# twitu/genome-assembly

Measured on NVIDIA B200. Metric: canonical k-mers binned+pruned per second, higher is better.
Workload: dtype u64

## Files before the change

genome-assembly_b200/csrc/bin3.cu:

```cuda
#include "bin3.cuh"
#include "gbin_device.cuh"
#include "gbin_internal.h"
#include "prefix_scan.cuh"

namespace gbin {


__device__ __forceinline__ uint32_t payload_bases(const uint32_t *pl, uint32_t nwords, uint32_t j, uint32_t h, bool rev) {
    const uint32_t bit = 2 * j, wi = bit >> 5, sh = bit & 31;
    const uint32_t a = wi < nwords ? pl[wi] : 0u, b = wi + 1 < nwords ? pl[wi + 1] : 0u;
    uint32_t x = __funnelshift_l(b, a, sh);
    if (rev) x = ~x;
    return h ? (x >> (32 - 2 * h)) : 0u;
}

template <int PW>
__global__ void __launch_bounds__(256)
    make_entries_kernel(const uint32_t *__restrict__ skr, uint64_t n_rec, KeyLayout kl, uint64_t *__restrict__ ent, uint16_t *__restrict__ piece_info,
                        unsigned long long *__restrict__ n_real) {
    constexpr int NW = SkrLayout<PW>::WORDS;
    const uint64_t i = (uint64_t)blockIdx.x * blockDim.x + threadIdx.x;
    uint32_t real = 0;
    if (i < n_rec) {
        const uint4 h = *reinterpret_cast<const uint4 *>(skr + i * NW);
// ... 293 lines not shown
                    emit(d - 1);
                    rnd++;
                    lo = d;
                    before += acc;
                    acc = 0;
                }
                acc += c;
            }
            emit(63);
            for (uint32_t j = rnd + 1; j < un.rounds; j++) {
                units[u + j].n_inst = 0;
                units[u + j].ibase = un.ibase + un.n_inst;
            }
            if (bad) atomicExch(&gc->overflow, 1u);
        }
        __syncwarp();
    }
}


struct UnitOut3 {
    uint32_t ibase;
    uint32_t S, N;
    uint32_t pad;
};

struct G3Stage {
    uint64_t *codes;
    uint32_t *mmer;
    uint32_t *loff;
    int32_t *ids;
    UnitOut3 *unit_out;
    uint64_t kmer_cap, id_cap;
    uint32_t kdiv;
};

template <int PW>
struct Payload {
    uint64_t w[PW];
    __device__ __forceinline__ void set(const uint4 &a, const uint4 &b) {
        w[0] = ((uint64_t)a.x << 32) | a.y;
        w[1] = ((uint64_t)a.z << 32) | a.w;
        if (PW == 4) {
            w[PW - 2] = ((uint64_t)b.x << 32) | b.y;
            w[PW - 1] = ((uint64_t)b.z << 32) | b.w;
        }
    }
    __device__ __forceinline__ void advance(uint32_t bases) {
        const uint32_t sh = 2 * bases;
#pragma unroll
        for (int q = 0; q < PW - 1; q++) w[q] = (w[q] << sh) | (w[q + 1] >> (64 - sh));
        w[PW - 1] <<= sh;
    }
    __device__ __forceinline__ void skip(uint32_t bases) {
        while (bases >= 31) {
            advance(31);
            bases -= 31;
        }
        if (bases) advance(bases);
    }
};

template <int PW, int KW>
__device__ __forceinline__ void front_kmer(const Payload<PW> &pl, int K, bool rev, uint64_t kmask0, uint64_t *k0, uint64_t *k1) {
    if (KW == 1) {
        uint64_t a = (2 * K == 64) ? pl.w[0] : (pl.w[0] >> (64 - 2 * K));
        if (rev) a = ~a & kmask0;
        *k0 = a;
        *k1 = 0;
    } else {
        const int r = 128 - 2 * K;
        uint64_t a = r ? (pl.w[0] >> r) : pl.w[0];
        uint64_t b = r ? ((pl.w[1] >> r) | (pl.w[0] << (64 - r))) : pl.w[1];
        if (rev) {
            a = ~a & kmask0;
            b = ~b;
        }
        *k0 = a;
        *k1 = b;
    }
}

template <int WCAP, int KW>
struct WarpLayout {
    static constexpr int NB_MAX = WCAP / 8;
    static constexpr int ECAP = WCAP / 4;
    static constexpr int BSTART_BYTES = ((NB_MAX + 1) * 2 + 15) / 16 * 16;
    static constexpr int BYTES = KW * WCAP * 8  + WCAP * 4  + WCAP * 2  + WCAP * 2  + WCAP * 2  + WCAP  + BSTART_BYTES +
                                 NB_MAX * 4  + ECAP * 4  + ECAP ;
};

__device__ __forceinline__ uint32_t warp_incl_scan_u32(uint32_t v, uint32_t lane) {
#pragma unroll
    for (int d = 1; d < 32; d <<= 1) {
        const uint32_t o = __shfl_up_sync(0xffffffffu, v, d);
        if (lane >= (uint32_t)d) v += o;
    }
    return v;
}

constexpr int G3_WARPS = 5;
constexpr uint32_t G3_SMALL_INST = 512, G3_SMALL_ENT = 128, G3_SMALL_NB = 64;

template <int PW, int KW, int WCAP, int WARPS, int U>
__global__ void __launch_bounds__(WARPS * 32)
    group3_kernel(const uint32_t *__restrict__ skr, const uint64_t *__restrict__ ent, const Unit3 *__restrict__ units, KeyLayout kl, int cutoff,
                  const int32_t *__restrict__ ids_by_arrival, int32_t id_base, G3Stage out, G3Counters *__restrict__ gc,
                  const uint32_t *__restrict__ chunk_bounds, uint32_t chunk, uint32_t *__restrict__ chunk_tickets, uint32_t size_class) {
    constexpr int NW = SkrLayout<PW>::WORDS;
    constexpr int HS = 2 * WCAP;
    constexpr int LOG_HS = WCAP == 512 ? 10 : 11;
    static_assert(WCAP == 512 || WCAP == 1024, "unit capacity");
    static_assert((1 << LOG_HS) == HS, "hash size");
    using WL = WarpLayout<WCAP, KW>;
    constexpr int NB_MAX = WL::NB_MAX, ECAP = WL::ECAP;
    extern __shared__ __align__(16) uint8_t smem3[];
    const uint32_t lane = threadIdx.x & 31, warp = threadIdx.x >> 5;
    uint8_t *wb = smem3 + (size_t)warp * WL::BYTES;
    uint64_t *key0 = reinterpret_cast<uint64_t *>(wb);
    uint64_t *key1 = key0 + (KW == 2 ? WCAP : 0);
    uint16_t *tbl16 = reinterpret_cast<uint16_t *>(key0 + KW * WCAP);
    uint32_t *cnt32 = reinterpret_cast<uint32_t *>(tbl16 + 2 * WCAP);
    uint16_t *cnt16 = reinterpret_cast<uint16_t *>(cnt32);
    uint16_t *grp = cnt16 + WCAP;
    uint16_t *rk = grp + WCAP;
    uint8_t *eix = reinterpret_cast<uint8_t *>(rk + WCAP);
    uint16_t *bstart = reinterpret_cast<uint16_t *>(eix + WCAP);
    uint32_t *bmm = reinterpret_cast<uint32_t *>(reinterpret_cast<uint8_t *>(bstart) + WL::BSTART_BYTES);
    int32_t *eid = reinterpret_cast<int32_t *>(bmm + NB_MAX);
    uint8_t *ebk = reinterpret_cast<uint8_t *>(eid + ECAP);
    uint16_t *surv = tbl16;
    uint16_t *sorted = surv + WCAP;
    int32_t *idbuf = reinterpret_cast<int32_t *>(tbl16);

    const int K = kl.K;
    const uint64_t kmask0 = (2 * K >= 64 * KW) ? ~0ull : ((1ull << (2 * K - 64 * (KW - 1))) - 1);
    const uint32_t unit_begin = chunk_bounds[chunk], unit_end = chunk_bounds[chunk + 1];
    const uint32_t lt_mask = (1u << lane) - 1u;
    const uint32_t cls_mask = (uint32_t)(kl.nc - 1);

    uint32_t u = 0;
    if (lane == 0) u = unit_begin + atomicAdd(&chunk_tickets[chunk], 1u);
    u = __shfl_sync(0xffffffffu, u, 0);
    while (u < unit_end) {
        Unit3 un;
        {
            const uint32_t wv = lane < 8 ? reinterpret_cast<const uint32_t *>(units + u)[lane] : 0u;
            un.ent_begin = __shfl_sync(0xffffffffu, wv, 0);
            un.ent_end = __shfl_sync(0xffffffffu, wv, 1);
            un.n_inst = __shfl_sync(0xffffffffu, wv, 2);
            un.round = __shfl_sync(0xffffffffu, wv, 3);
            un.rounds = __shfl_sync(0xffffffffu, wv, 4);
            un.drange = __shfl_sync(0xffffffffu, wv, 5);
            un.ibase = __shfl_sync(0xffffffffu, wv, 6);
        }
        uint32_t u_next = 0;
        if (lane == 0) u_next = unit_begin + atomicAdd(&chunk_tickets[chunk], 1u);
        const uint32_t u_cur = u;
        const bool is_round = un.rounds != 0;
        const uint32_t n_ent = un.ent_end - un.ent_begin;
        const bool packed = !is_round && n_ent <= (uint32_t)ECAP;
        if (size_class) {
            const bool small = !is_round && un.n_inst <= G3_SMALL_INST && n_ent <= G3_SMALL_ENT;
            if (small != (size_class == 1u)) {
                u = __shfl_sync(0xffffffffu, u_next, 0);
                continue;
            }
        }
        if (is_round && un.n_inst == 0) {
            if (lane == 0) out.unit_out[u_cur] = UnitOut3{un.ibase, 0u, 0u, 0u};
            u = __shfl_sync(0xffffffffu, u_next, 0);
            continue;
        }

        {
            uint4 *z = reinterpret_cast<uint4 *>(tbl16);
            for (uint32_t i = lane; i < (uint32_t)(WCAP * 4 + WCAP * 2) / 16; i += 32) z[i] = make_uint4(0u, 0u, 0u, 0u);
        }
        __syncwarp();

        int dlo = 0, dhi = 63;
        const uint32_t ibase = un.ibase;
        bool bad = false;
        if (is_round) {
            dlo = (int)(un.drange & 0xffu);
            dhi = (int)((un.drange >> 8) & 0xffu);
        }

        uint32_t n_inst = 0, n_bkt = 0;
        if (!bad) {
            uint32_t carry_pos = 0, carry_ord = 0, prev_mm = 0xffffffffu;
            for (uint32_t e0 = 0; e0 < n_ent; e0 += 32) {
                const uint32_t e = e0 + lane;
                uint32_t np = 0, t0 = 0, mm = 0xffffffffu, arrival = 0;
                bool rev = false;
                uint4 ha = make_uint4(0u, 0u, 0u, 0u), pa = ha, pb = ha;
                if (e < n_ent) {
                    const uint64_t en = ent[un.ent_begin + e];
                    const uint32_t slot = (uint32_t)en;
                    mm = (uint32_t)(en >> 32) >> kl.mshift;
                    const uint4 *rp = reinterpret_cast<const uint4 *>(skr + (uint64_t)(slot >> kl.cshift) * NW);
                    ha = rp[0];
                    pa = rp[1];
                    if (PW == 4) pb = rp[2];
                    arrival = ha.x;
                    const uint32_t meta = ha.z;
                    rev = (meta >> 8) & 1u;
                    piece_of(meta, slot & cls_mask, kl, &t0, &np);
                    if (is_round && np) {
                        const int so = (int)((meta >> 16) & 0xffu);
                        int a = so - dhi, b = so - dlo;
                        if (a < (int)t0) a = (int)t0;
                        if (b > (int)(t0 + np - 1)) b = (int)(t0 + np - 1);
                        if (dlo > dhi || b < a) np = 0;
                        else {
                            t0 = (uint32_t)a;
                            np = (uint32_t)(b - a + 1);
                        }
                    }
                }
                uint32_t pm = __shfl_up_sync(0xffffffffu, mm, 1);
                if (lane == 0) pm = prev_mm;
                const bool head = e < n_ent && mm != pm;
                const uint32_t hs = warp_incl_scan_u32(head ? 1u : 0u, lane);
                const uint32_t ps = warp_incl_scan_u32(np, lane);
                const uint32_t ord = carry_ord + hs - 1;
                const uint32_t pos0 = carry_pos + ps - np;
                if (head && ord < (uint32_t)NB_MAX) {
                    bstart[ord] = (uint16_t)pos0;
                    bmm[ord] = mm;
                }
                carry_ord += __shfl_sync(0xffffffffu, hs, 31);
                carry_pos += __shfl_sync(0xffffffffu, ps, 31);
                prev_mm = __shfl_sync(0xffffffffu, mm, 31);
                if (carry_pos > (uint32_t)WCAP || carry_ord > (uint32_t)NB_MAX || (!packed && carry_ord > 1u)) {
                    bad = true;
                    break;
                }
                if (packed && e < n_ent) {
                    eid[e] = ids_by_arrival ? ids_by_arrival[arrival] : id_base + (int32_t)arrival;
                    ebk[e] = (uint8_t)ord;
                }
                if (np) {
                    Payload<PW> pl;
                    pl.set(pa, pb);
                    pl.skip(t0);
                    for (uint32_t i = 0; i < np; i++) {
                        uint64_t k0, k1;
                        front_kmer<PW, KW>(pl, K, rev, kmask0, &k0, &k1);
                        key0[pos0 + i] = k0;
                        if (KW == 2) key1[pos0 + i] = k1;
                        if (packed) eix[pos0 + i] = (uint8_t)e;
                        pl.advance(1);
                    }
                }
            }
            n_inst = carry_pos;
            n_bkt = carry_ord;
            if (!bad && lane == 0) bstart[n_bkt] = (uint16_t)n_inst;
        }
        __syncwarp();
        if (bad) {
            if (lane == 0) {
                atomicExch(&gc->overflow, 1u);
                out.unit_out[u_cur] = UnitOut3{ibase, 0u, 0u, 0u};
            }
            u = __shfl_sync(0xffffffffu, u_next, 0);
            continue;
        }

        for (uint32_t b0 = 0; b0 < n_inst; b0 += 32 * U) {
            uint64_t k0[U], k1[U];
            uint32_t lo[U], hi[U], idx[U], rep[U], cur[U];
            bool valid[U];
#pragma unroll
            for (int j = 0; j < U; j++) {
                const uint32_t p = b0 + j * 32 + lane;
                valid[j] = p < n_inst;
                k0[j] = valid[j] ? key0[p] : 0ull;
                k1[j] = (KW == 2 && valid[j]) ? key1[p] : 0ull;
                uint32_t o = 0;
                if (packed && valid[j]) o = ebk[eix[p]];
                lo[j] = bstart[o];
                hi[j] = bstart[o + 1];
                uint32_t hx = ((uint32_t)k0[j] * 0x9E3779B1u) ^ ((uint32_t)(k0[j] >> 32) * 0x85EBCA77u) ^ (o * 0xC2B2AE3Du);
                if (KW == 2) hx ^= ((uint32_t)k1[j] * 0x27D4EB2Fu) ^ ((uint32_t)(k1[j] >> 32) * 0x165667B1u);
                hx *= 0x9E3779B1u;
                idx[j] = hx >> (32 - LOG_HS);
                rep[j] = 0xffffffffu;
            }
#pragma unroll
            for (int j = 0; j < U; j++) cur[j] = valid[j] ? tbl16[idx[j]] : 0u;
#pragma unroll
            for (int j = 0; j < U; j++) {
                if (valid[j] && cur[j] == 0) {
                    const uint32_t p = b0 + j * 32 + lane;
                    const uint32_t old = atomicCAS(&tbl16[idx[j]], (unsigned short)0, (unsigned short)(p + 1));
                    if (old == 0) rep[j] = p;
                    else cur[j] = old;
                }
            }
#pragma unroll
            for (int j = 0; j < U; j++) {
                if (valid[j] && rep[j] == 0xffffffffu) {
                    const uint32_t r = cur[j] - 1;
                    if (r >= lo[j] && r < hi[j] && key0[r] == k0[j] && (KW == 1 || key1[r] == k1[j])) rep[j] = r;
                }
            }
#pragma unroll
            for (int j = 0; j < U; j++) {
                if (valid[j] && rep[j] == 0xffffffffu) {
                    const uint32_t p = b0 + j * 32 + lane;
                    uint32_t ix = (idx[j] + 1) & (HS - 1);
                    for (;;) {
                        uint32_t c = tbl16[ix];
                        if (c == 0) {
                            c = atomicCAS(&tbl16[ix], (unsigned short)0, (unsigned short)(p + 1));
                            if (c == 0) {
                                rep[j] = p;
                                break;
                            }
                        }
                        const uint32_t r = c - 1;
                        if (r >= lo[j] && r < hi[j] && key0[r] == k0[j] && (KW == 1 || key1[r] == k1[j])) {
                            rep[j] = r;
                            break;
                        }
                        ix = (ix + 1) & (HS - 1);
                    }
                }
            }
            unsigned peers[U];
            uint32_t c[U];
#pragma unroll
            for (int j = 0; j < U; j++) peers[j] = __match_any_sync(0xffffffffu, valid[j] ? rep[j] : (0x10000u + lane));
#pragma unroll
            for (int j = 0; j < U; j++) {
                c[j] = 0;
                if (valid[j] && (int)lane == __ffs(peers[j]) - 1) {
                    const uint32_t sh = 16u * (rep[j] & 1u);
                    c[j] = (atomicAdd(&cnt32[rep[j] >> 1], (uint32_t)__popc(peers[j]) << sh) >> sh) & 0xffffu;
                }
                __syncwarp();
            }
#pragma unroll
            for (int j = 0; j < U; j++) {
                c[j] = __shfl_sync(0xffffffffu, c[j], __ffs(peers[j]) - 1);
                if (valid[j]) {
                    const uint32_t p = b0 + j * 32 + lane;
                    grp[p] = (uint16_t)rep[j];
                    rk[p] = (uint16_t)(c[j] + __popc(peers[j] & lt_mask));
                }
            }
        }
        __syncwarp();

        uint32_t S = 0, N = 0, D = 0;
        for (uint32_t b0 = 0; b0 < n_inst; b0 += 32 * U) {
            bool leader[U];
            uint32_t c[U];
#pragma unroll
            for (int j = 0; j < U; j++) {
                const uint32_t p = b0 + j * 32 + lane;
                leader[j] = p < n_inst && grp[p] == p;
            }
#pragma unroll
            for (int j = 0; j < U; j++) c[j] = leader[j] ? cnt16[b0 + j * 32 + lane] : 0u;
#pragma unroll
            for (int j = 0; j < U; j++) {
                const uint32_t p = b0 + j * 32 + lane;
                const bool sv = leader[j] && (cutoff < 0 || c[j] > (uint32_t)cutoff);
                const unsigned lm = __ballot_sync(0xffffffffu, leader[j]), sm = __ballot_sync(0xffffffffu, sv);
                if (sv) surv[S + __popc(sm & lt_mask)] = (uint16_t)p;
                else if (leader[j]) cnt16[p] = 0xffffu;
                S += __popc(sm);
                D += __popc(lm);
                N += sv ? c[j] : 0u;
            }
        }
#pragma unroll
        for (int d = 16; d > 0; d >>= 1) N += __shfl_xor_sync(0xffffffffu, N, d);
        const uint64_t kbase = ibase / out.kdiv;
        const bool oob = (uint64_t)ibase + N > out.id_cap || kbase + S > out.kmer_cap;
        if (lane == 0) {
            out.unit_out[u_cur] = UnitOut3{ibase, oob ? 0u : S, oob ? 0u : N, 0u};
            atomicAdd(&gc->distinct, (unsigned long long)D);
            if (oob) atomicExch(&gc->overflow, 2u);
        }
        __syncwarp();
        if (oob) {
            u = __shfl_sync(0xffffffffu, u_next, 0);
            continue;
        }

        for (uint32_t x0 = 0; x0 < S; x0 += 32) {
            const uint32_t x = x0 + lane;
            if (x < S) {
                const uint32_t p = surv[x];
                uint32_t a = 0, a2 = S;
                if (n_bkt > 1) {
                    const uint32_t o = ebk[eix[p]];
                    const uint32_t blo = bstart[o], bhi = bstart[o + 1];
                    uint32_t b = S;
                    while (a < b) {
                        const uint32_t m = (a + b) >> 1;
                        if (surv[m] < blo) a = m + 1;
                        else b = m;
                    }
                    uint32_t b2 = S;
                    a2 = a;
                    while (a2 < b2) {
                        const uint32_t m = (a2 + b2) >> 1;
                        if (surv[m] < bhi) a2 = m + 1;
                        else b2 = m;
                    }
                }
                const uint64_t k0 = key0[p], k1 = (KW == 2) ? key1[p] : 0ull;
                uint32_t rank = a;
                for (uint32_t t = a; t < a2; t++) {
                    const uint32_t q = surv[t];
                    const uint64_t q0 = key0[q];
                    bool less = q0 < k0;
                    if constexpr (KW == 2) less = less || (q0 == k0 && key1[q] < k1);
                    rank += less ? 1u : 0u;
                }
                sorted[rank] = (uint16_t)p;
            }
        }
        __syncwarp();

        {
            uint32_t carry = 0;
            for (uint32_t x0 = 0; x0 < S; x0 += 32) {
                const uint32_t x = x0 + lane;
                const uint32_t p = x < S ? sorted[x] : 0u;
                const uint32_t c = x < S ? cnt16[p] : 0u;
                const uint32_t inc = warp_incl_scan_u32(c, lane);
                if (x < S) cnt16[p] = (uint16_t)(carry + inc);
                carry += __shfl_sync(0xffffffffu, inc, 31);
            }
        }
        __syncwarp();

        for (uint32_t x0 = 0; x0 < S; x0 += 32) {
            const uint32_t x = x0 + lane;
            if (x < S) {
                const uint32_t p = sorted[x];
                const uint32_t beg = x ? cnt16[sorted[x - 1]] : 0u;
                const uint64_t g = kbase + x;
                out.codes[g * KW] = key0[p];
                if (KW == 2) out.codes[g * KW + 1] = key1[p];
                out.mmer[g] = bmm[n_bkt > 1 ? ebk[eix[p]] : 0u];
                out.loff[g] = beg;
            }
        }
        __syncwarp();

        if (N) {
            if (packed) {
                for (uint32_t b0 = 0; b0 < n_inst; b0 += 32 * U) {
                    uint32_t end[U], r[U];
                    int32_t id[U];
#pragma unroll
                    for (int j = 0; j < U; j++) {
                        const uint32_t p = b0 + j * 32 + lane;
                        end[j] = 0xffffu;
                        r[j] = 0;
                        id[j] = 0;
                        if (p < n_inst) {
                            end[j] = cnt16[grp[p]];
                            r[j] = rk[p];
                            id[j] = eid[eix[p]];
                        }
                    }
#pragma unroll
                    for (int j = 0; j < U; j++)
                        if (end[j] != 0xffffu) idbuf[end[j] - 1u - r[j]] = id[j];
                }
            } else {
                uint32_t carry_pos = 0;
                for (uint32_t e0 = 0; e0 < n_ent; e0 += 32) {
                    const uint32_t e = e0 + lane;
                    uint32_t np = 0, arrival = 0;
                    if (e < n_ent) {
                        const uint32_t slot = (uint32_t)ent[un.ent_begin + e];
                        const uint32_t *rec = skr + (uint64_t)(slot >> kl.cshift) * NW;
                        const uint32_t meta = rec[2];
                        arrival = rec[0];
                        uint32_t t0;
                        piece_of(meta, slot & cls_mask, kl, &t0, &np);
                        if (is_round && np) {
                            const int so = (int)((meta >> 16) & 0xffu);
                            int a = so - dhi, b = so - dlo;
                            if (a < (int)t0) a = (int)t0;
                            if (b > (int)(t0 + np - 1)) b = (int)(t0 + np - 1);
                            np = (dlo > dhi || b < a) ? 0u : (uint32_t)(b - a + 1);
                        }
                    }
                    const uint32_t ps = warp_incl_scan_u32(np, lane);
                    const uint32_t pos0 = carry_pos + ps - np;
                    carry_pos += __shfl_sync(0xffffffffu, ps, 31);
                    if (np) {
                        const int32_t id = ids_by_arrival ? ids_by_arrival[arrival] : id_base + (int32_t)arrival;
                        for (uint32_t i = 0; i < np; i++) {
                            const uint32_t p = pos0 + i;
                            const uint32_t end = cnt16[grp[p]];
                            if (end != 0xffffu) idbuf[end - 1u - rk[p]] = id;
                        }
                    }
                }
            }
            __syncwarp();
            int32_t *dst = out.ids + ibase;
            for (uint32_t i = lane; i < N; i += 32) dst[i] = idbuf[i];
        }
        __syncwarp();
        u = __shfl_sync(0xffffffffu, u_next, 0);
    }
}


struct UnitSN {
    const UnitOut3 *uo;
    const uint32_t *chunk_bounds;
    uint32_t chunk;
    __device__ __forceinline__ uint64_t operator()(uint64_t u) const {
        if (u < chunk_bounds[chunk] || u >= chunk_bounds[chunk + 1]) return 0ull;
        return ((uint64_t)uo[u].S << 32) | uo[u].N;
    }
};

__global__ void v3_chunk_total_kernel(const uint64_t *__restrict__ chunk_sum, uint32_t chunk, unsigned long long *__restrict__ totals, G3Counters *__restrict__ gc,
                                      uint32_t n_chunks, int which) {
    const unsigned long long t = (chunk ? totals[chunk - 1] : 0ull) + *chunk_sum;
    totals[chunk] = t;
    if (chunk + 1 == n_chunks) {
        if (which == 0) {
            gc->total_kmers = t >> 32;
            gc->total_ids = t & 0xffffffffull;
        } else {
            gc->lsd_kmers = t >> 32;
            gc->lsd_ids = t & 0xffffffffull;
        }
    }
}

struct G3Final {
    uint64_t *kmer_codes;
    uint32_t *kmer_mmer;
    uint64_t *kmer_id_off;
    int32_t *read_ids;
    uint64_t id_off_base;
};

struct G3Lsd {
    const uint64_t *excl;
    void *rec;
    uint32_t *src_off;
    uint32_t *cnt;
    uint32_t *fidx;
    uint32_t *nadj;
    uint64_t cap;
};

struct UnitSNLong {
    const UnitOut3 *uo;
    const Unit3 *units;
    const uint32_t *chunk_bounds;
    uint32_t chunk;
    __device__ __forceinline__ uint64_t operator()(uint64_t u) const {
        if (u < chunk_bounds[chunk] || u >= chunk_bounds[chunk + 1]) return 0ull;
        const uint32_t sl = units[u].span_len;
        if (sl != SPAN_MEMBER_LONG && (sl <= SPAN_SHORT_MAX || sl == SPAN_MEMBER)) return 0ull;
        return ((uint64_t)uo[u].S << 32) | uo[u].N;
    }
};

template <int KW>
__device__ __forceinline__ void finalize3_unit(const Unit3 *__restrict__ units, const uint64_t *__restrict__ unit_excl, unsigned long long base,
                                               unsigned long long lsd_base, const G3Stage &st, const G3Final &fin, const G3Lsd &ls, G3Counters *gc, uint32_t u,
                                               uint32_t lane, bool only_long) {
    const uint32_t span_len = units[u].span_len;
    if (only_long && span_len != SPAN_MEMBER_LONG && (span_len <= SPAN_SHORT_MAX || span_len == SPAN_MEMBER)) return;
    const uint64_t ex = unit_excl[u];
    const UnitOut3 uo = st.unit_out[u];
    const uint64_t Sb = (base >> 32) + (ex >> 32), Nb = (base & 0xffffffffull) + (ex & 0xffffffffull);
    if (span_len == 0) {
        const uint64_t kb = uo.ibase / st.kdiv;
        for (uint32_t x0 = 0; x0 < uo.S; x0 += 128) {
            uint64_t c0[4], c1[4];
            uint32_t mm[4], lo[4];
#pragma unroll
            for (int q = 0; q < 4; q++) {
                const uint32_t x = x0 + q * 32 + lane;
                if (x < uo.S) {
                    c0[q] = st.codes[(kb + x) * KW];
                    if (KW == 2) c1[q] = st.codes[(kb + x) * KW + 1];
                    mm[q] = st.mmer[kb + x];
                    lo[q] = st.loff[kb + x];
                }
// ... 130 lines not shown
__global__ void lsd_place_kernel(const Rec<KW> *__restrict__ rec, uint64_t n, const uint64_t *__restrict__ dnew, G3Lsd ls, G3Final fin) {
    const uint64_t q = (uint64_t)blockIdx.x * blockDim.x + threadIdx.x;
    if (q >= n) return;
    const Rec<KW> r = load_rec<KW>(rec + q);
    const uint64_t f = ls.fidx[q];
    fin.kmer_codes[f * KW] = r.k[0];
    if (KW == 2) fin.kmer_codes[f * KW + 1] = r.k[KW - 1];
    fin.kmer_mmer[f] = r.mmer;
    fin.kmer_id_off[f] = fin.id_off_base + dnew[q] + ls.nadj[q];
}

template <int KW>
__global__ void __launch_bounds__(256)
    lsd_lists_kernel(const Rec<KW> *__restrict__ rec, uint64_t n, const uint64_t *__restrict__ dnew, G3Lsd ls, const int32_t *__restrict__ stg_ids, G3Final fin) {
    const uint64_t q = ((uint64_t)blockIdx.x * blockDim.x + threadIdx.x) >> 3;
    if (q >= n) return;
    const uint32_t p = rec[q].arrival;
    const uint32_t c = ls.cnt[p];
    const int32_t *src = stg_ids + ls.src_off[p];
    int32_t *dst = fin.read_ids + dnew[q] + ls.nadj[q];
    for (uint32_t i = threadIdx.x & 7u; i < c; i += 8) dst[i] = src[i];
}

__global__ void v3_chunk_bounds_kernel(const Unit3 *__restrict__ units, const G3Counters *__restrict__ gc, uint32_t n_chunks, uint32_t *__restrict__ chunk_bounds) {
    const uint32_t nu = gc->n_units;
    for (uint32_t c = 0; c <= n_chunks; c++) {
        uint32_t b = (uint32_t)(((uint64_t)nu * c) / n_chunks);
        if (c == n_chunks) b = nu;
        else {
            while (b > 0 && b < nu && (units[b].span_len == SPAN_MEMBER || units[b].span_len == SPAN_MEMBER_LONG)) b--;
        }
        chunk_bounds[c] = b;
    }
}


static bool v3_hybrid(const KeyLayout &kl, int cap_i) { return cap_i != 512 && kl.K <= 32; }
static Plan3 v3_plan_params(const KeyLayout &kl, int cap_i) {
    const uint32_t cap = cap_i == 512 ? 512u : 1024u;
    Plan3 pp{cap, cap / 8, cap / 4, (uint32_t)(kl.K - kl.M + 1), cap, cap / 8, cap / 4};
    if (v3_hybrid(kl, cap_i)) {
        pp.cap_s = G3_SMALL_INST;
        pp.nb_s = G3_SMALL_NB;
        pp.ecap_s = G3_SMALL_ENT;
    }
    return pp;
}

uint64_t v3_max_units(uint64_t n_inst, uint64_t n_runs, int cap) {
    const uint64_t c = cap == 512 ? 512 : 1024;
    return n_runs + 5 * (n_inst / c) + 16;
}
size_t v3_unit_bytes() { return sizeof(Unit3); }
size_t v3_unit_out_bytes() { return sizeof(UnitOut3); }

struct PtrIn64 {
    const uint64_t *p;
    __device__ __forceinline__ uint64_t operator()(uint64_t j) const { return p[j]; }
};

int v3_plan_units(const uint16_t *sorted_info, const uint64_t *ent, const KeyLayout &kl, int cap, const uint32_t *inst_prefix, const uint32_t *run_start, uint64_t n_runs,
                  uint64_t *nunits64, uint64_t *base64, uint32_t *atom3, uint32_t *spanlen, uint32_t *head_run, void *scratch, void *units, uint64_t max_units,
                  void *gc_dev, uint32_t n_chunks, uint32_t *chunk_bounds, cudaStream_t st) {
    RunView3 rv{run_start, inst_prefix};
    const Plan3 pp = v3_plan_params(kl, cap);
    G3Counters *gc = static_cast<G3Counters *>(gc_dev);
    cudaMemsetAsync(gc, 0, sizeof(G3Counters), st);
    int l = 0;
    if (n_runs) {
        uint32_t *atom_c = atom3, *atom_e = atom3 + n_runs, *atom_mm = atom3 + 2 * n_runs;
        v3_atoms_kernel<<<(unsigned)((n_runs + 255) / 256), 256, 0, st>>>(rv, ent, n_runs, kl.mshift, atom_c, atom_e, atom_mm);
        const uint64_t walkers = (n_runs + PLAN_BLOCK - 1) / PLAN_BLOCK;
        v3_pack_kernel<<<(unsigned)((walkers + 127) / 128), 128, 0, st>>>(atom_c, atom_e, atom_mm, n_runs, pp, nunits64, spanlen);
        l += 2 + exclusive_scan<uint64_t, PtrIn64>(PtrIn64{nunits64}, base64, n_runs, static_cast<uint64_t *>(scratch), base64 + n_runs, st);
        v3_head_runs_kernel<<<(unsigned)((n_runs + 255) / 256), 256, 0, st>>>(nunits64, base64, n_runs, head_run);
        v3_fill_units_kernel<<<(unsigned)((max_units + 255) / 256), 256, 0, st>>>(rv, nunits64, spanlen, base64, base64 + n_runs, n_runs, head_run, static_cast<Unit3 *>(units), gc);
        v3_round_cuts_kernel<<<592, 128, 0, st>>>(sorted_info, static_cast<Unit3 *>(units), gc, pp.cap);
        l += 3;
    }
    v3_chunk_bounds_kernel<<<1, 1, 0, st>>>(static_cast<const Unit3 *>(units), gc, n_chunks, chunk_bounds);
    return l + 1;
}

size_t v3_group_smem_bytes(int KW, int cap) {
    const size_t per_warp = cap == 512 ? (KW == 1 ? WarpLayout<512, 1>::BYTES : WarpLayout<512, 2>::BYTES)
                                       : (KW == 1 ? WarpLayout<1024, 1>::BYTES : WarpLayout<1024, 2>::BYTES);
    return per_warp * G3_WARPS;
}

int v3_group_launch(const void *skr, const uint64_t *ent, const void *units, const KeyLayout &kl, int cap, int cutoff, const int32_t *ids_by_arrival, int32_t id_base,
                    const V3Out &o, uint64_t max_units, uint64_t *unit_excl, uint64_t *lsd_excl, void *scan_scratch, void *gc_dev, const V3Chunks &ch, const V3Lsd &lsd,
                    bool finalize_only, int sm_count, KernelProf *prof, cudaStream_t st) {
    const int KW = kl.K <= 32 ? 1 : 2;
    constexpr int WARPS = G3_WARPS;
    const size_t smem = v3_group_smem_bytes(KW, cap);
    cudaMemsetAsync(ch.tickets, 0, sizeof(uint32_t) * 2 * ch.n, st);
    const uint32_t kdiv = cutoff >= 0 ? (uint32_t)cutoff + 1u : 1u;
    G3Stage stg{o.stg_codes, o.stg_mmer, o.stg_loff, o.stg_ids, static_cast<UnitOut3 *>(o.unit_out), o.kmer_cap, o.id_cap, kdiv};
    G3Final fin{o.kmer_codes, o.kmer_mmer, o.kmer_id_off, o.read_ids, o.id_off_base};
    G3Lsd ls{lsd_excl, lsd.rec, lsd.src_off, lsd.cnt, lsd.fidx, lsd.nadj, lsd.cap};
    G3Counters *gc = static_cast<G3Counters *>(gc_dev);
    const uint32_t *sk = static_cast<const uint32_t *>(skr);
    const Unit3 *un = static_cast<const Unit3 *>(units);
    int per_sm = (int)((size_t)(227 * 1024) / (smem + 1024));
    if (per_sm < 1) per_sm = 1;
    const bool hybrid = v3_hybrid(kl, cap);
    const size_t smem_s = v3_group_smem_bytes(KW, 512);
    int per_sm_s = (int)((size_t)(227 * 1024) / (smem_s + 1024));
    if (per_sm_s < 1) per_sm_s = 1;
    int launches = 0;
    auto launch = [&](auto kern, auto kern_small, auto fin_kern) {
        cudaFuncSetAttribute(kern, cudaFuncAttributeMaxDynamicSharedMemorySize, (int)smem);
        if (hybrid) cudaFuncSetAttribute(kern_small, cudaFuncAttributeMaxDynamicSharedMemorySize, (int)smem_s);
        for (uint32_t c = 0; c < ch.n; c++) {
            if (!finalize_only) {
                bool on = prof && prof->begin(KK_SKR_GROUP, st);
                if (!hybrid) {
                    kern<<<sm_count * per_sm, WARPS * 32, smem, st>>>(sk, ent, un, kl, cutoff, ids_by_arrival, id_base, stg, gc, ch.bounds, c, ch.tickets, 0u);
                } else {
                    cudaEventRecord(ch.ev_fork, st);
                    cudaStreamWaitEvent(ch.aux, ch.ev_fork, 0);
                    kern<<<sm_count * 2, WARPS * 32, smem, st>>>(sk, ent, un, kl, cutoff, ids_by_arrival, id_base, stg, gc, ch.bounds, c, ch.tickets, 2u);
                    kern_small<<<sm_count * per_sm_s, WARPS * 32, smem_s, ch.aux>>>(sk, ent, un, kl, cutoff, ids_by_arrival, id_base, stg, gc, ch.bounds, c, ch.tickets + ch.n, 1u);
                    cudaEventRecord(ch.ev_join, ch.aux);
                    cudaStreamWaitEvent(st, ch.ev_join, 0);
                }
                if (prof) prof->end(on, hybrid ? 2 : 1, st);
                launches += hybrid ? 2 : 1;
            }
            bool on = prof && prof->begin(KK_V3_SPAN, st);
            int l = exclusive_scan<uint64_t, UnitSN>(UnitSN{stg.unit_out, ch.bounds, c}, unit_excl, max_units, static_cast<uint64_t *>(scan_scratch), ch.chunk_sum, st);
            v3_chunk_total_kernel<<<1, 1, 0, st>>>(ch.chunk_sum, c, ch.totals_dev, gc, ch.n, 0);
            l += exclusive_scan<uint64_t, UnitSNLong>(UnitSNLong{stg.unit_out, un, ch.bounds, c}, lsd_excl, max_units, static_cast<uint64_t *>(scan_scratch), ch.chunk_sum, st);
            v3_chunk_total_kernel<<<1, 1, 0, st>>>(ch.chunk_sum, c, ch.lsd_totals_dev, gc, ch.n, 1);
            fin_kern<<<sm_count * 12, 128, 0, st>>>(un, unit_excl, ch.totals_dev, ch.lsd_totals_dev, stg, fin, ls, gc, ch.bounds, c, finalize_only);
            if (prof) prof->end(on, l + 3, st);
            launches += l + 3;
            if (ch.totals_host) {
                cudaMemcpyAsync(ch.totals_host + c, ch.totals_dev + c, sizeof(unsigned long long), cudaMemcpyDeviceToHost, st);
                cudaMemcpyAsync(ch.lsd_totals_host + c, ch.lsd_totals_dev + c, sizeof(unsigned long long), cudaMemcpyDeviceToHost, st);
            }
            if (ch.done) cudaEventRecord(ch.done[c], st);
        }
    };
    if (KW == 1) {
        if (cap == 512) launch(group3_kernel<2, 1, 512, WARPS, 2>, group3_kernel<2, 1, 512, WARPS, 2>, finalize3_kernel<1>);
        else launch(group3_kernel<2, 1, 1024, WARPS, 4>, group3_kernel<2, 1, 512, WARPS, 2>, finalize3_kernel<1>);
    } else {
        if (cap == 512) launch(group3_kernel<4, 2, 512, WARPS, 2>, group3_kernel<4, 2, 512, WARPS, 2>, finalize3_kernel<2>);
        else launch(group3_kernel<4, 2, 1024, WARPS, 4>, group3_kernel<4, 2, 512, WARPS, 2>, finalize3_kernel<2>);
    }
    return launches;
}

template <int KW>
struct RecHead {
    const Rec<KW> *rec;
    __device__ __forceinline__ uint32_t operator()(uint64_t p) const { return (p == 0 || rec[p].mmer != rec[p - 1].mmer) ? 1u : 0u; }
};
template <int KW>
__global__ void span_starts_kernel(const Rec<KW> *__restrict__ rec, uint64_t n, const uint32_t *__restrict__ idx, uint32_t *__restrict__ starts,
                                   uint32_t *__restrict__ n_spans, uint32_t *__restrict__ flag) {
    const uint64_t p = (uint64_t)blockIdx.x * blockDim.x + threadIdx.x;
    if (p >= n) return;
    const bool head = p == 0 || rec[p].mmer != rec[p - 1].mmer;
    if (head) starts[idx[p]] = (uint32_t)p;
    if (p == n - 1) {
        const uint32_t total = idx[p] + (head ? 1u : 0u);
        starts[total] = (uint32_t)n;
        *n_spans = total;
        *flag = 0u;
    }
}

constexpr int SS_RMAX = 1024;
template <int KW, int CAP, int THREADS>
__global__ void __launch_bounds__(THREADS)
    span_sort_kernel(Rec<KW> *__restrict__ rec, const uint32_t *__restrict__ starts, const uint32_t *__restrict__ n_spans_ptr, uint32_t m_min, uint32_t m_max,
                     uint32_t *__restrict__ too_big) {
    extern __shared__ __align__(16) uint8_t ss_smem[];
    uint64_t *ka = reinterpret_cast<uint64_t *>(ss_smem);
    uint64_t *kb = ka + KW * CAP;
    uint16_t *sa = reinterpret_cast<uint16_t *>(kb + KW * CAP);
    uint16_t *sb = sa + CAP;
    uint16_t *ra = sb + CAP;
    uint16_t *rb = ra + SS_RMAX + 2;
    __shared__ uint32_t s_nruns;
    const uint32_t tid = threadIdx.x, lane = tid & 31;
    const uint32_t n_spans = *n_spans_ptr;
    for (uint32_t s = blockIdx.x; s < n_spans; s += gridDim.x) {
        const uint32_t b = starts[s], m = starts[s + 1] - b;
        if (m < m_min) continue;
        if (m > m_max) continue;
        const uint32_t mmer = rec[b].mmer;
        for (uint32_t i = tid; i < m; i += THREADS) {
            const Rec<KW> r = load_rec<KW>(rec + b + i);
            ka[i] = r.k[0];
            if (KW == 2) ka[CAP + i] = r.k[KW - 1];
            sa[i] = (uint16_t)i;
        }
        __syncthreads();
        if (tid < 32) {
            uint32_t nr = 0;
            for (uint32_t i0 = 0; i0 < m; i0 += 32) {
                const uint32_t i = i0 + lane;
                bool head = false;
                if (i < m) {
                    head = i == 0 || ka[i] < ka[i - 1];
                    if (KW == 2 && i && ka[i] == ka[i - 1]) head = ka[CAP + i] < ka[CAP + i - 1];
                }
                const unsigned bal = __ballot_sync(0xffffffffu, head);
                if (head) {
                    const uint32_t pos = nr + __popc(bal & ((1u << lane) - 1u));
                    if (pos < (uint32_t)SS_RMAX) ra[pos] = (uint16_t)i;
                }
                nr += __popc(bal);
            }
            if (lane == 0) {
                s_nruns = nr;
                if (nr <= (uint32_t)SS_RMAX) ra[nr] = (uint16_t)m;
            }
        }
        __syncthreads();
        uint32_t nr = s_nruns;
        if (nr > (uint32_t)SS_RMAX) {
            if (tid == 0) atomicExch(too_big, 1u);
            __syncthreads();
            continue;
        }
        uint64_t *src_k = ka, *dst_k = kb;
        uint16_t *src_s = sa, *dst_s = sb, *src_r = ra, *dst_r = rb;
        while (nr > 1) {
            for (uint32_t i = tid; i < m; i += THREADS) {
// ... 307 lines not shown
```

Baseline: 23.41 billion.

## Process 1024-capacity group units with warp pairs instead of single warps

For the 1024-instance unit capacity, each unit is now handled by two cooperating warps synchronised with named barriers. Cross-warp scans and totals go through a small shared exchange buffer, and each warp keeps its own count table that is merged later. The hybrid large-class launch also changes from a fixed two CTAs per SM to the occupancy-derived CTA count. This aims to cut per-unit latency and raise parallelism on large units, at the cost of extra barriers, a second count table in shared memory, and fewer units per CTA.

```diff
diff --git a/genome-assembly_b200/csrc/bin3.cu b/genome-assembly_b200/csrc/bin3.cu
--- a/genome-assembly_b200/csrc/bin3.cu
+++ b/genome-assembly_b200/csrc/bin3.cu
@@ -399,12 +399,14 @@
 }
 
 template <int WCAP, int KW>
-struct WarpLayout {
+struct UnitLayout {
+    static constexpr int W = WCAP == 1024 ? 2 : 1;
     static constexpr int NB_MAX = WCAP / 8;
     static constexpr int ECAP = WCAP / 4;
     static constexpr int BSTART_BYTES = ((NB_MAX + 1) * 2 + 15) / 16 * 16;
-    static constexpr int BYTES = KW * WCAP * 8  + WCAP * 4  + WCAP * 2  + WCAP * 2  + WCAP * 2  + WCAP  + BSTART_BYTES +
-                                 NB_MAX * 4  + ECAP * 4  + ECAP ;
+    static constexpr int XCH_BYTES = W == 2 ? 64 : 0;
+    static constexpr int BYTES = KW * WCAP * 8  + WCAP * 4  + W * WCAP * 2  + WCAP * 2  + WCAP * 2  + WCAP  +
+                                 BSTART_BYTES + NB_MAX * 4  + ECAP * 4  + ECAP  + XCH_BYTES;
 };
 
 __device__ __forceinline__ uint32_t warp_incl_scan_u32(uint32_t v, uint32_t lane) {
@@ -416,36 +418,83 @@
     return v;
 }
 
+template <int W>
+__device__ __forceinline__ void unit_sync(uint32_t bar_id) {
+    if (W == 1) __syncwarp();
+    else asm volatile("bar.sync %0, 64;" ::"r"(bar_id) : "memory");
+}
+
+struct PairXch {
+    uint32_t *x;
+    uint32_t slot;
+    __device__ __forceinline__ const uint32_t *put(uint32_t h, uint32_t lane, uint32_t bar_id, uint32_t a, uint32_t b = 0u, uint32_t c = 0u) {
+        uint32_t *s = x + slot * 8;
+        if (lane == 0) {
+            s[h * 4] = a;
+            s[h * 4 + 1] = b;
+            s[h * 4 + 2] = c;
+        }
+        slot ^= 1u;
+        unit_sync<2>(bar_id);
+        return s;
+    }
+};
+
+template <int W>
+__device__ __forceinline__ uint32_t unit_incl_scan(uint32_t v, uint32_t lane, uint32_t h, uint32_t bar_id, PairXch &xc, uint32_t *total) {
+    v = warp_incl_scan_u32(v, lane);
+    const uint32_t wt = __shfl_sync(0xffffffffu, v, 31);
+    if (W == 1) {
+        *total = wt;
+        return v;
+    }
+    const uint32_t *s = xc.put(h, lane, bar_id, wt);
+    *total = s[0] + s[4];
+    return v + (h ? s[0] : 0u);
+}
+
 constexpr int G3_WARPS = 5;
+constexpr int G3_PAIRS = 3;
+constexpr int g3_ctas_per_sm(size_t smem) {
+    const int n = (int)((size_t)(227 * 1024) / (smem + 1024));
+    return n > 1 ? n : 1;
+}
 constexpr uint32_t G3_SMALL_INST = 512, G3_SMALL_ENT = 128, G3_SMALL_NB = 64;
 
-template <int PW, int KW, int WCAP, int WARPS, int U>
-__global__ void __launch_bounds__(WARPS * 32)
+template <int PW, int KW, int WCAP, int UNITS, int U>
+__global__ void __launch_bounds__(UNITS * UnitLayout<WCAP, KW>::W * 32, WCAP == 1024 ? g3_ctas_per_sm(UNITS * UnitLayout<WCAP, KW>::BYTES) : 0)
     group3_kernel(const uint32_t *__restrict__ skr, const uint64_t *__restrict__ ent, const Unit3 *__restrict__ units, KeyLayout kl, int cutoff,
                   const int32_t *__restrict__ ids_by_arrival, int32_t id_base, G3Stage out, G3Counters *__restrict__ gc,
                   const uint32_t *__restrict__ chunk_bounds, uint32_t chunk, uint32_t *__restrict__ chunk_tickets, uint32_t size_class) {
+    using WL = UnitLayout<WCAP, KW>;
+    constexpr int W = WL::W;
     constexpr int NW = SkrLayout<PW>::WORDS;
     constexpr int HS = 2 * WCAP;
     constexpr int LOG_HS = WCAP == 512 ? 10 : 11;
     static_assert(WCAP == 512 || WCAP == 1024, "unit capacity");
     static_assert((1 << LOG_HS) == HS, "hash size");
-    using WL = WarpLayout<WCAP, KW>;
     constexpr int NB_MAX = WL::NB_MAX, ECAP = WL::ECAP;
     extern __shared__ __align__(16) uint8_t smem3[];
     const uint32_t lane = threadIdx.x & 31, warp = threadIdx.x >> 5;
-    uint8_t *wb = smem3 + (size_t)warp * WL::BYTES;
+    const uint32_t h = warp % W, bar_id = 1 + warp / W;
+    const uint32_t ul = h * 32 + lane;
+    const bool first = ul == 0;
+    uint8_t *wb = smem3 + (size_t)(warp / W) * WL::BYTES;
     uint64_t *key0 = reinterpret_cast<uint64_t *>(wb);
     uint64_t *key1 = key0 + (KW == 2 ? WCAP : 0);
     uint16_t *tbl16 = reinterpret_cast<uint16_t *>(key0 + KW * WCAP);
     uint32_t *cnt32 = reinterpret_cast<uint32_t *>(tbl16 + 2 * WCAP);
     uint16_t *cnt16 = reinterpret_cast<uint16_t *>(cnt32);
-    uint16_t *grp = cnt16 + WCAP;
+    uint32_t *cntlo32 = cnt32 + (W - 1) * WCAP / 2;
+    uint16_t *cntlo16 = reinterpret_cast<uint16_t *>(cntlo32);
+    uint16_t *grp = cnt16 + W * WCAP;
     uint16_t *rk = grp + WCAP;
     uint8_t *eix = reinterpret_cast<uint8_t *>(rk + WCAP);
     uint16_t *bstart = reinterpret_cast<uint16_t *>(eix + WCAP);
     uint32_t *bmm = reinterpret_cast<uint32_t *>(reinterpret_cast<uint8_t *>(bstart) + WL::BSTART_BYTES);
     int32_t *eid = reinterpret_cast<int32_t *>(bmm + NB_MAX);
     uint8_t *ebk = reinterpret_cast<uint8_t *>(eid + ECAP);
+    PairXch xc{reinterpret_cast<uint32_t *>(ebk + ECAP), 0u};
     uint16_t *surv = tbl16;
     uint16_t *sorted = surv + WCAP;
     int32_t *idbuf = reinterpret_cast<int32_t *>(tbl16);
@@ -455,10 +504,14 @@
     const uint32_t unit_begin = chunk_bounds[chunk], unit_end = chunk_bounds[chunk + 1];
     const uint32_t lt_mask = (1u << lane) - 1u;
     const uint32_t cls_mask = (uint32_t)(kl.nc - 1);
+    auto share_ticket = [&](uint32_t t) -> uint32_t {
+        if (W == 1) return __shfl_sync(0xffffffffu, t, 0);
+        return xc.put(h, lane, bar_id, __shfl_sync(0xffffffffu, t, 0))[0];
+    };
 
     uint32_t u = 0;
-    if (lane == 0) u = unit_begin + atomicAdd(&chunk_tickets[chunk], 1u);
-    u = __shfl_sync(0xffffffffu, u, 0);
+    if (first) u = unit_begin + atomicAdd(&chunk_tickets[chunk], 1u);
+    u = share_ticket(u);
     while (u < unit_end) {
         Unit3 un;
         {
@@ -472,7 +525,7 @@
             un.ibase = __shfl_sync(0xffffffffu, wv, 6);
         }
         uint32_t u_next = 0;
-        if (lane == 0) u_next = unit_begin + atomicAdd(&chunk_tickets[chunk], 1u);
+        if (first) u_next = unit_begin + atomicAdd(&chunk_tickets[chunk], 1u);
         const uint32_t u_cur = u;
         const bool is_round = un.rounds != 0;
         const uint32_t n_ent = un.ent_end - un.ent_begin;
@@ -480,21 +533,21 @@
         if (size_class) {
             const bool small = !is_round && un.n_inst <= G3_SMALL_INST && n_ent <= G3_SMALL_ENT;
             if (small != (size_class == 1u)) {
-                u = __shfl_sync(0xffffffffu, u_next, 0);
+                u = share_ticket(u_next);
                 continue;
             }
         }
         if (is_round && un.n_inst == 0) {
-            if (lane == 0) out.unit_out[u_cur] = UnitOut3{un.ibase, 0u, 0u, 0u};
-            u = __shfl_sync(0xffffffffu, u_next, 0);
+            if (first) out.unit_out[u_cur] = UnitOut3{un.ibase, 0u, 0u, 0u};
+            u = share_ticket(u_next);
             continue;
         }
 
         {
             uint4 *z = reinterpret_cast<uint4 *>(tbl16);
-            for (uint32_t i = lane; i < (uint32_t)(WCAP * 4 + WCAP * 2) / 16; i += 32) z[i] = make_uint4(0u, 0u, 0u, 0u);
-        }
-        __syncwarp();
+            for (uint32_t i = ul; i < (uint32_t)(WCAP * 4 + W * WCAP * 2) / 16; i += 32 * W) z[i] = make_uint4(0u, 0u, 0u, 0u);
+        }
+        unit_sync<W>(bar_id);
 
         int dlo = 0, dhi = 63;
         const uint32_t ibase = un.ibase;
@@ -507,8 +560,8 @@
         uint32_t n_inst = 0, n_bkt = 0;
         if (!bad) {
             uint32_t carry_pos = 0, carry_ord = 0, prev_mm = 0xffffffffu;
-            for (uint32_t e0 = 0; e0 < n_ent; e0 += 32) {
-                const uint32_t e = e0 + lane;
+            for (uint32_t e0 = 0; e0 < n_ent; e0 += 32 * W) {
+                const uint32_t e = e0 + ul;
                 uint32_t np = 0, t0 = 0, mm = 0xffffffffu, arrival = 0;
                 bool rev = false;
                 uint4 ha = make_uint4(0u, 0u, 0u, 0u), pa = ha, pb = ha;
@@ -537,19 +590,32 @@
                     }
                 }
                 uint32_t pm = __shfl_up_sync(0xffffffffu, mm, 1);
-                if (lane == 0) pm = prev_mm;
+                if (lane == 0) {
+                    if (W == 1) pm = prev_mm;
+                    else pm = (e == 0 || e >= n_ent) ? 0xffffffffu : (uint32_t)(ent[un.ent_begin + e - 1] >> 32) >> kl.mshift;
+                }
                 const bool head = e < n_ent && mm != pm;
-                const uint32_t hs = warp_incl_scan_u32(head ? 1u : 0u, lane);
-                const uint32_t ps = warp_incl_scan_u32(np, lane);
+                uint32_t hs = warp_incl_scan_u32(head ? 1u : 0u, lane);
+                uint32_t ps = warp_incl_scan_u32(np, lane);
+                uint32_t hs_all = __shfl_sync(0xffffffffu, hs, 31), ps_all = __shfl_sync(0xffffffffu, ps, 31);
+                if (W == 2) {
+                    const uint32_t *s = xc.put(h, lane, bar_id, hs_all, ps_all);
+                    if (h) {
+                        hs += s[0];
+                        ps += s[1];
+                    }
+                    hs_all = s[0] + s[4];
+                    ps_all = s[1] + s[5];
+                }
                 const uint32_t ord = carry_ord + hs - 1;
                 const uint32_t pos0 = carry_pos + ps - np;
                 if (head && ord < (uint32_t)NB_MAX) {
                     bstart[ord] = (uint16_t)pos0;
                     bmm[ord] = mm;
                 }
-                carry_ord += __shfl_sync(0xffffffffu, hs, 31);
-                carry_pos += __shfl_sync(0xffffffffu, ps, 31);
-                prev_mm = __shfl_sync(0xffffffffu, mm, 31);
+                carry_ord += hs_all;
+                carry_pos += ps_all;
+                if (W == 1) prev_mm = __shfl_sync(0xffffffffu, mm, 31);
                 if (carry_pos > (uint32_t)WCAP || carry_ord > (uint32_t)NB_MAX || (!packed && carry_ord > 1u)) {
                     bad = true;
                     break;
@@ -574,26 +640,29 @@
             }
             n_inst = carry_pos;
             n_bkt = carry_ord;
-            if (!bad && lane == 0) bstart[n_bkt] = (uint16_t)n_inst;
-        }
-        __syncwarp();
+            if (!bad && first) bstart[n_bkt] = (uint16_t)n_inst;
+        }
+        unit_sync<W>(bar_id);
         if (bad) {
-            if (lane == 0) {
+            if (first) {
                 atomicExch(&gc->overflow, 1u);
                 out.unit_out[u_cur] = UnitOut3{ibase, 0u, 0u, 0u};
             }
-            u = __shfl_sync(0xffffffffu, u_next, 0);
+            u = share_ticket(u_next);
             continue;
         }
-
-        for (uint32_t b0 = 0; b0 < n_inst; b0 += 32 * U) {
+        const uint32_t mid = W == 1 ? n_inst : min(n_inst, (n_inst + 63) / 64 * 32);
+        const uint32_t pbeg = h ? mid : 0u, pend = h ? n_inst : mid;
+
+        uint32_t *cntw32 = (W == 2 && h == 0) ? cntlo32 : cnt32;
+        for (uint32_t b0 = pbeg; b0 < pend; b0 += 32 * U) {
             uint64_t k0[U], k1[U];
             uint32_t lo[U], hi[U], idx[U], rep[U], cur[U];
             bool valid[U];
 #pragma unroll
             for (int j = 0; j < U; j++) {
                 const uint32_t p = b0 + j * 32 + lane;
-                valid[j] = p < n_inst;
+                valid[j] = p < pend;
                 k0[j] = valid[j] ? key0[p] : 0ull;
                 k1[j] = (KW == 2 && valid[j]) ? key1[p] : 0ull;
                 uint32_t o = 0;
@@ -656,7 +725,7 @@
                 c[j] = 0;
                 if (valid[j] && (int)lane == __ffs(peers[j]) - 1) {
                     const uint32_t sh = 16u * (rep[j] & 1u);
-                    c[j] = (atomicAdd(&cnt32[rep[j] >> 1], (uint32_t)__popc(peers[j]) << sh) >> sh) & 0xffffu;
+                    c[j] = (atomicAdd(&cntw32[rep[j] >> 1], (uint32_t)__popc(peers[j]) << sh) >> sh) & 0xffffu;
                 }
                 __syncwarp();
             }
@@ -670,26 +739,29 @@
                 }
             }
         }
-        __syncwarp();
+        unit_sync<W>(bar_id);
 
         uint32_t S = 0, N = 0, D = 0;
-        for (uint32_t b0 = 0; b0 < n_inst; b0 += 32 * U) {
+        uint16_t *my_surv = h ? sorted : surv;
+        for (uint32_t b0 = pbeg; b0 < pend; b0 += 32 * U) {
             bool leader[U];
             uint32_t c[U];
 #pragma unroll
             for (int j = 0; j < U; j++) {
                 const uint32_t p = b0 + j * 32 + lane;
-                leader[j] = p < n_inst && grp[p] == p;
-            }
-#pragma unroll
-            for (int j = 0; j < U; j++) c[j] = leader[j] ? cnt16[b0 + j * 32 + lane] : 0u;
+                leader[j] = p < pend && grp[p] == p;
+            }
+#pragma unroll
+            for (int j = 0; j < U; j++) c[j] = leader[j] ? cnt16[b0 + j * 32 + lane] + (W == 2 ? cntlo16[b0 + j * 32 + lane] : 0u) : 0u;
 #pragma unroll
             for (int j = 0; j < U; j++) {
                 const uint32_t p = b0 + j * 32 + lane;
                 const bool sv = leader[j] && (cutoff < 0 || c[j] > (uint32_t)cutoff);
                 const unsigned lm = __ballot_sync(0xffffffffu, leader[j]), sm = __ballot_sync(0xffffffffu, sv);
-                if (sv) surv[S + __popc(sm & lt_mask)] = (uint16_t)p;
-                else if (leader[j]) cnt16[p] = 0xffffu;
+                if (sv) {
+                    my_surv[S + __popc(sm & lt_mask)] = (uint16_t)p;
+                    if (W == 2) cnt16[p] = (uint16_t)c[j];
+                } else if (leader[j]) cnt16[p] = 0xffffu;
                 S += __popc(sm);
                 D += __popc(lm);
                 N += sv ? c[j] : 0u;
@@ -697,21 +769,33 @@
         }
 #pragma unroll
         for (int d = 16; d > 0; d >>= 1) N += __shfl_xor_sync(0xffffffffu, N, d);
+        uint32_t S_lo = S;
+        if (W == 2) {
+            const uint32_t *s = xc.put(h, lane, bar_id, S, N, D);
+            S_lo = s[0];
+            S = s[0] + s[4];
+            N = s[1] + s[5];
+            D = s[2] + s[6];
+        }
         const uint64_t kbase = ibase / out.kdiv;
         const bool oob = (uint64_t)ibase + N > out.id_cap || kbase + S > out.kmer_cap;
-        if (lane == 0) {
+        if (first) {
             out.unit_out[u_cur] = UnitOut3{ibase, oob ? 0u : S, oob ? 0u : N, 0u};
             atomicAdd(&gc->distinct, (unsigned long long)D);
             if (oob) atomicExch(&gc->overflow, 2u);
         }
-        __syncwarp();
         if (oob) {
-            u = __shfl_sync(0xffffffffu, u_next, 0);
+            u = share_ticket(u_next);
             continue;
         }
-
-        for (uint32_t x0 = 0; x0 < S; x0 += 32) {
-            const uint32_t x = x0 + lane;
+        if (W == 2 && h) {
+            __syncwarp();
+            for (uint32_t x = lane; x < S - S_lo; x += 32) surv[S_lo + x] = sorted[x];
+        }
+        unit_sync<W>(bar_id);
+
+        for (uint32_t x0 = 0; x0 < S; x0 += 32 * W) {
+            const uint32_t x = x0 + ul;
             if (x < S) {
                 const uint32_t p = surv[x];
                 uint32_t a = 0, a2 = S;
@@ -744,23 +828,24 @@
                 sorted[rank] = (uint16_t)p;
             }
         }
-        __syncwarp();
+        unit_sync<W>(bar_id);
 
         {
             uint32_t carry = 0;
-            for (uint32_t x0 = 0; x0 < S; x0 += 32) {
-                const uint32_t x = x0 + lane;
+            for (uint32_t x0 = 0; x0 < S; x0 += 32 * W) {
+                const uint32_t x = x0 + ul;
                 const uint32_t p = x < S ? sorted[x] : 0u;
                 const uint32_t c = x < S ? cnt16[p] : 0u;
-                const uint32_t inc = warp_incl_scan_u32(c, lane);
+                uint32_t all;
+                const uint32_t inc = unit_incl_scan<W>(c, lane, h, bar_id, xc, &all);
                 if (x < S) cnt16[p] = (uint16_t)(carry + inc);
-                carry += __shfl_sync(0xffffffffu, inc, 31);
-            }
-        }
-        __syncwarp();
-
-        for (uint32_t x0 = 0; x0 < S; x0 += 32) {
-            const uint32_t x = x0 + lane;
+                carry += all;
+            }
+        }
+        unit_sync<W>(bar_id);
+
+        for (uint32_t x0 = 0; x0 < S; x0 += 32 * W) {
+            const uint32_t x = x0 + ul;
             if (x < S) {
                 const uint32_t p = sorted[x];
                 const uint32_t beg = x ? cnt16[sorted[x - 1]] : 0u;
@@ -771,11 +856,11 @@
                 out.loff[g] = beg;
             }
         }
-        __syncwarp();
+        unit_sync<W>(bar_id);
 
         if (N) {
             if (packed) {
-                for (uint32_t b0 = 0; b0 < n_inst; b0 += 32 * U) {
+                for (uint32_t b0 = pbeg; b0 < pend; b0 += 32 * U) {
                     uint32_t end[U], r[U];
                     int32_t id[U];
 #pragma unroll
@@ -784,9 +869,10 @@
                         end[j] = 0xffffu;
                         r[j] = 0;
                         id[j] = 0;
-                        if (p < n_inst) {
-                            end[j] = cnt16[grp[p]];
-                            r[j] = rk[p];
+                        if (p < pend) {
+                            const uint32_t g = grp[p];
+                            end[j] = cnt16[g];
+                            r[j] = rk[p] + (W == 2 && h ? cntlo16[g] : 0u);
                             id[j] = eid[eix[p]];
                         }
                     }
@@ -796,8 +882,8 @@
                 }
             } else {
                 uint32_t carry_pos = 0;
-                for (uint32_t e0 = 0; e0 < n_ent; e0 += 32) {
-                    const uint32_t e = e0 + lane;
+                for (uint32_t e0 = 0; e0 < n_ent; e0 += 32 * W) {
+                    const uint32_t e = e0 + ul;
                     uint32_t np = 0, arrival = 0;
                     if (e < n_ent) {
                         const uint32_t slot = (uint32_t)ent[un.ent_begin + e];
@@ -814,25 +900,27 @@
                             np = (dlo > dhi || b < a) ? 0u : (uint32_t)(b - a + 1);
                         }
                     }
-                    const uint32_t ps = warp_incl_scan_u32(np, lane);
+                    uint32_t all;
+                    const uint32_t ps = unit_incl_scan<W>(np, lane, h, bar_id, xc, &all);
                     const uint32_t pos0 = carry_pos + ps - np;
-                    carry_pos += __shfl_sync(0xffffffffu, ps, 31);
+                    carry_pos += all;
                     if (np) {
                         const int32_t id = ids_by_arrival ? ids_by_arrival[arrival] : id_base + (int32_t)arrival;
                         for (uint32_t i = 0; i < np; i++) {
                             const uint32_t p = pos0 + i;
-                            const uint32_t end = cnt16[grp[p]];
-                            if (end != 0xffffu) idbuf[end - 1u - rk[p]] = id;
+                            const uint32_t g = grp[p];
+                            const uint32_t end = cnt16[g];
+                            if (end != 0xffffu) idbuf[end - 1u - rk[p] - (W == 2 && p >= mid ? cntlo16[g] : 0u)] = id;
                         }
                     }
                 }
             }
-            __syncwarp();
+            unit_sync<W>(bar_id);
             int32_t *dst = out.ids + ibase;
-            for (uint32_t i = lane; i < N; i += 32) dst[i] = idbuf[i];
-        }
-        __syncwarp();
-        u = __shfl_sync(0xffffffffu, u_next, 0);
+            for (uint32_t i = ul; i < N; i += 32 * W) dst[i] = idbuf[i];
+        }
+        if (W == 1) __syncwarp();
+        u = share_ticket(u_next);
     }
 }
 
@@ -1129,18 +1217,21 @@
     return l + 1;
 }
 
+static int v3_group_units(int cap) { return cap == 512 ? G3_WARPS : G3_PAIRS; }
+static int v3_group_threads(int cap) { return v3_group_units(cap) * (cap == 512 ? UnitLayout<512, 1>::W : UnitLayout<1024, 1>::W) * 32; }
+
 size_t v3_group_smem_bytes(int KW, int cap) {
-    const size_t per_warp = cap == 512 ? (KW == 1 ? WarpLayout<512, 1>::BYTES : WarpLayout<512, 2>::BYTES)
-                                       : (KW == 1 ? WarpLayout<1024, 1>::BYTES : WarpLayout<1024, 2>::BYTES);
-    return per_warp * G3_WARPS;
+    const size_t per_unit = cap == 512 ? (KW == 1 ? UnitLayout<512, 1>::BYTES : UnitLayout<512, 2>::BYTES)
+                                       : (KW == 1 ? UnitLayout<1024, 1>::BYTES : UnitLayout<1024, 2>::BYTES);
+    return per_unit * v3_group_units(cap);
 }
 
 int v3_group_launch(const void *skr, const uint64_t *ent, const void *units, const KeyLayout &kl, int cap, int cutoff, const int32_t *ids_by_arrival, int32_t id_base,
                     const V3Out &o, uint64_t max_units, uint64_t *unit_excl, uint64_t *lsd_excl, void *scan_scratch, void *gc_dev, const V3Chunks &ch, const V3Lsd &lsd,
                     bool finalize_only, int sm_count, KernelProf *prof, cudaStream_t st) {
     const int KW = kl.K <= 32 ? 1 : 2;
-    constexpr int WARPS = G3_WARPS;
     const size_t smem = v3_group_smem_bytes(KW, cap);
+    const int threads = v3_group_threads(cap), threads_s = v3_group_threads(512);
     cudaMemsetAsync(ch.tickets, 0, sizeof(uint32_t) * 2 * ch.n, st);
     const uint32_t kdiv = cutoff >= 0 ? (uint32_t)cutoff + 1u : 1u;
     G3Stage stg{o.stg_codes, o.stg_mmer, o.stg_loff, o.stg_ids, static_cast<UnitOut3 *>(o.unit_out), o.kmer_cap, o.id_cap, kdiv};
@@ -1149,12 +1240,10 @@
     G3Counters *gc = static_cast<G3Counters *>(gc_dev);
     const uint32_t *sk = static_cast<const uint32_t *>(skr);
     const Unit3 *un = static_cast<const Unit3 *>(units);
-    int per_sm = (int)((size_t)(227 * 1024) / (smem + 1024));
-    if (per_sm < 1) per_sm = 1;
+    const int per_sm = g3_ctas_per_sm(smem);
     const bool hybrid = v3_hybrid(kl, cap);
     const size_t smem_s = v3_group_smem_bytes(KW, 512);
-    int per_sm_s = (int)((size_t)(227 * 1024) / (smem_s + 1024));
-    if (per_sm_s < 1) per_sm_s = 1;
+    const int per_sm_s = g3_ctas_per_sm(smem_s);
     int launches = 0;
     auto launch = [&](auto kern, auto kern_small, auto fin_kern) {
         cudaFuncSetAttribute(kern, cudaFuncAttributeMaxDynamicSharedMemorySize, (int)smem);
@@ -1163,12 +1252,12 @@
             if (!finalize_only) {
                 bool on = prof && prof->begin(KK_SKR_GROUP, st);
                 if (!hybrid) {
-                    kern<<<sm_count * per_sm, WARPS * 32, smem, st>>>(sk, ent, un, kl, cutoff, ids_by_arrival, id_base, stg, gc, ch.bounds, c, ch.tickets, 0u);
+                    kern<<<sm_count * per_sm, threads, smem, st>>>(sk, ent, un, kl, cutoff, ids_by_arrival, id_base, stg, gc, ch.bounds, c, ch.tickets, 0u);
                 } else {
                     cudaEventRecord(ch.ev_fork, st);
                     cudaStreamWaitEvent(ch.aux, ch.ev_fork, 0);
-                    kern<<<sm_count * 2, WARPS * 32, smem, st>>>(sk, ent, un, kl, cutoff, ids_by_arrival, id_base, stg, gc, ch.bounds, c, ch.tickets, 2u);
-                    kern_small<<<sm_count * per_sm_s, WARPS * 32, smem_s, ch.aux>>>(sk, ent, un, kl, cutoff, ids_by_arrival, id_base, stg, gc, ch.bounds, c, ch.tickets + ch.n, 1u);
+                    kern<<<sm_count * per_sm, threads, smem, st>>>(sk, ent, un, kl, cutoff, ids_by_arrival, id_base, stg, gc, ch.bounds, c, ch.tickets, 2u);
+                    kern_small<<<sm_count * per_sm_s, threads_s, smem_s, ch.aux>>>(sk, ent, un, kl, cutoff, ids_by_arrival, id_base, stg, gc, ch.bounds, c, ch.tickets + ch.n, 1u);
                     cudaEventRecord(ch.ev_join, ch.aux);
                     cudaStreamWaitEvent(st, ch.ev_join, 0);
                 }
@@ -1190,12 +1279,13 @@
             if (ch.done) cudaEventRecord(ch.done[c], st);
         }
     };
+    constexpr int W5 = G3_WARPS, P3 = G3_PAIRS;
     if (KW == 1) {
-        if (cap == 512) launch(group3_kernel<2, 1, 512, WARPS, 2>, group3_kernel<2, 1, 512, WARPS, 2>, finalize3_kernel<1>);
-        else launch(group3_kernel<2, 1, 1024, WARPS, 4>, group3_kernel<2, 1, 512, WARPS, 2>, finalize3_kernel<1>);
+        if (cap == 512) launch(group3_kernel<2, 1, 512, W5, 2>, group3_kernel<2, 1, 512, W5, 2>, finalize3_kernel<1>);
+        else launch(group3_kernel<2, 1, 1024, P3, 4>, group3_kernel<2, 1, 512, W5, 2>, finalize3_kernel<1>);
     } else {
-        if (cap == 512) launch(group3_kernel<4, 2, 512, WARPS, 2>, group3_kernel<4, 2, 512, WARPS, 2>, finalize3_kernel<2>);
-        else launch(group3_kernel<4, 2, 1024, WARPS, 4>, group3_kernel<4, 2, 512, WARPS, 2>, finalize3_kernel<2>);
+        if (cap == 512) launch(group3_kernel<4, 2, 512, W5, 2>, group3_kernel<4, 2, 512, W5, 2>, finalize3_kernel<2>);
+        else launch(group3_kernel<4, 2, 1024, P3, 4>, group3_kernel<4, 2, 512, W5, 2>, finalize3_kernel<2>);
     }
     return launches;
 }
```

New measurement: 24.24 billion, median of 6. +3.5%, better.
